# ssheybani/baby-vision-curriculum

Hardware: AMD Instinct MI355X
Metric: video clips/sec (node) VideoMAE-base 16x224^2 bf16 pretraining (higher is better)
Workload: dtype bf16; 1 GPU; VideoMAE-base (ViT-B/16 encoder, 4-layer decoder), 16x224x224 clips, tubelet 2, 90% tube mask, full training step (fwd + MSE + bwd + GradScaler + SGD-Nesterov); clips_per_gpu=256, global_batch=256, parallelism=dp1, weights=random init N(0,0.02), seed 0

## Files before the change

__graft_entry__.py:

```python
import importlib.util
import os
import subprocess
import sys

ROOT = os.path.dirname(os.path.abspath(__file__))
PKG_DIR = os.path.join(ROOT, "baby-vision-curriculum_amd")
CSRC = os.path.join(PKG_DIR, "csrc")
LIB = os.path.join(PKG_DIR, "libbvc_hip.so")
PRODUCT_SOURCES = ["gemm.hip", "gemm_persist.hip", "gemm8.hip", "gemm_as.hip", "attention.hip", "attention_probs.hip", "rowops.hip", "stack.hip", "videomae.hip", "jepa.hip", "comm.hip"]
EXPERIMENT_SOURCES = [os.path.join("experiments", "gemm_big.hip"), os.path.join("experiments", "gemm_pp.hip")]
EXPERIMENT_INCLUDES = [os.path.join("experiments", "attention_dq_wave96.inc")]
HEADERS = ["common.h", "dropgate.h", "gemm.h", "gemm_tile.h", "gemm_kernel_body.inc", "attention.h", "attention_fwd_body.inc", "attention_dq_body.inc", "attention_dkdv_body.inc", "rowops.h", "stack.h", os.path.join("..", "..", "include", "bvc.h")]


def _experiments():
    return "BVC_EXPERIMENTS" in os.environ.get("BVC_EXTRA_HIPCC_FLAGS", "")


def _sources():
    return PRODUCT_SOURCES + (EXPERIMENT_SOURCES if _experiments() else [])


SOURCES = PRODUCT_SOURCES


EXPERIMENT_FLAGS = {"attention.hip": ["-mllvm", "-amdgpu-mfma-vgpr-form=1"]}


def _extra_flags(src):
    return EXPERIMENT_FLAGS.get(src, []) if _experiments() else []


HASH_FILE = LIB + ".srchash"


def _source_hash():
    import hashlib
    h = hashlib.sha256()
    for f in _sources() + HEADERS + (EXPERIMENT_INCLUDES if _experiments() else []):
        with open(os.path.join(CSRC, f), "rb") as fh:
            h.update(f.encode() + b"\0" + fh.read())
    h.update(os.environ.get("BVC_EXTRA_HIPCC_FLAGS", "").encode())
    return h.hexdigest()


def _stale():
    if not (os.path.exists(LIB) and os.path.exists(HASH_FILE)):
        return True
    with open(HASH_FILE) as fh:
        return fh.read().strip() != _source_hash()


def _hash_of(files):
    import hashlib
    h = hashlib.sha256()
    for f in files:
        with open(os.path.join(CSRC, f), "rb") as fh:
            h.update(f.encode() + b"\0" + fh.read())
    return h.hexdigest()


def build(force: bool = False) -> None:
    if force or _stale():
        from concurrent.futures import ThreadPoolExecutor
        hipcc = os.environ.get("HIPCC", "/opt/rocm/bin/hipcc")
        objdir = os.path.join(PKG_DIR, "build")
        os.makedirs(objdir, exist_ok=True)
        flags = ["--offload-arch=gfx950", "-O3", "-std=c++17", "-fPIC"] + os.environ.get("BVC_EXTRA_HIPCC_FLAGS", "").split()

        def compile_one(src):
            obj = os.path.join(objdir, os.path.basename(src).replace(".hip", ".o"))
            stamp = obj + ".hash"
            fl = flags + _extra_flags(src) + ["-I" + CSRC]
            want = _hash_of([src] + HEADERS + (EXPERIMENT_INCLUDES if _experiments() else [])) + " " + " ".join(fl)
            if not force and os.path.exists(obj) and os.path.exists(stamp) and open(stamp).read() == want:
                return obj
            cmd = [hipcc, *fl, "-c", os.path.join(CSRC, src), "-o", obj]
            if src == "gemm8.hip":
                r = subprocess.run(cmd + ["-Rpass-analysis=kernel-resource-usage"], stderr=subprocess.PIPE, text=True)
                if r.returncode != 0:
                    sys.stderr.write(r.stderr)
                    raise subprocess.CalledProcessError(r.returncode, cmd)
                name = None
                for line in r.stderr.splitlines():
                    if "Function Name:" in line:
                        name = line.split("Function Name:")[1].split()[0]
                    elif "VGPRs Spill:" in line and name and "gemm8_kernel" in name and name.endswith("ELi0EEEvNS_9GemmGroupEi"):
                        if int(line.split("VGPRs Spill:")[1].split()[0]) != 0:
                            raise RuntimeError(f"gemm8.hip: {name} spills VGPRs; its counted-wait epilogue assumes none")
            else:
                subprocess.run(cmd, check=True)
            with open(stamp, "w") as fh:
                fh.write(want)
            return obj

        srcs = _sources()
        with ThreadPoolExecutor(max_workers=min(8, len(srcs))) as ex:
            objs = list(ex.map(compile_one, srcs))
        subprocess.run([hipcc, "--offload-arch=gfx950", "-shared", "-fPIC", *objs, "-o", LIB], check=True)
        with open(HASH_FILE, "w") as fh:
            fh.write(_source_hash())
    pkg = load_package()
    pkg._lib.lib()


def load_package():
    if "bvc_amd" in sys.modules:
        return sys.modules["bvc_amd"]
    spec = importlib.util.spec_from_file_location("bvc_amd", os.path.join(PKG_DIR, "__init__.py"),
                                                  submodule_search_locations=[PKG_DIR])
    mod = importlib.util.module_from_spec(spec)
    sys.modules["bvc_amd"] = mod
    spec.loader.exec_module(mod)
    return mod


def smoke() -> None:
    import torch
    if ROOT not in sys.path:
        sys.path.insert(0, ROOT)
    from oracle import videomae_oracle as vo
    build()
    bvc = load_package()
    cfg = vo.TINY
    params = vo.make_params(cfg, seed=0)
    pixels, mask = vo.synthetic_batch(cfg, 2, seed=0, mask_ratio=0.75)
    ref_loss, ref_grads = vo.step(cfg, params, pixels, mask)

    dev = torch.device("cuda:0")
    model = bvc.VideoMAEForPreTraining(bvc.VideoMAEConfig(**{k: v for k, v in cfg.__dict__.items() if k != "decoder_norm_eps"}))
    model.load_state_dict(params)
    model.to(dev).train()
    out = model(pixels.to(dev), bool_masked_pos=mask.to(dev))
    out.loss.backward()
    torch.cuda.synchronize()
    loss = float(out.loss)
    rel = abs(loss - float(ref_loss)) / abs(float(ref_loss))
    assert rel < 2e-3, f"smoke: loss {loss} vs oracle {float(ref_loss)} (rel {rel:.2e})"
    for name in vo.GRAD_PROBES:
        g = dict(model.named_parameters())[name].grad.float().cpu()
        r = ref_grads[name]
        e = float((g - r).norm() / r.norm())
        assert e < 3e-2, f"smoke: grad {name} rel err {e:.2e}"
    print(f"smoke ok: loss {loss:.6f} (oracle {float(ref_loss):.6f}, rel {rel:.1e})")


if __name__ == "__main__":
    build(force="--force" in sys.argv)
    if "--smoke" in sys.argv:
        smoke()
```

baby-vision-curriculum_amd/csrc/attention.hip:

```cpp
#include <stdlib.h>

#include "attention.h"

namespace bvc {

#define AS3 __attribute__((address_space(3)))
#define MFMA32(a, b, c) __builtin_amdgcn_mfma_f32_32x32x16_bf16((a), (b), (c), 0, 0, 0)

template <int HD>
__device__ __forceinline__ int swz_dual(int r) {
    if constexpr (HD == 64) return (((r >> 1) & 1) << 2) | ((r >> 2) & 3);
    else return (r >> 2) & 3;
}

template <int HD>
constexpr int pan_w(int p) { return HD - 64 * p >= 64 ? 64 : HD - 64 * p; }
constexpr int img_hd(int hd) { return hd == 80 || hd == 88 ? 96 : hd; }
constexpr uint32_t kDmaZero = 0xfffffff0u;
__device__ __forceinline__ int swz_pw(int pw, int r) { return pw == 64 ? swz_dual<64>(r) : swz_dual<32>(r); }

template <int PW, int NW, int VC = PW / 8>
__device__ __forceinline__ void stage_panel(__amdgpu_buffer_rsrc_t rs, int row0, int ld, int col0, char* lds, int GB, int wave, int lane) {
    constexpr int CPR = PW / 8;
    constexpr int RPP = 64 / CPR;
#pragma unroll
    for (int jj = 0; jj < (PW / 8 + NW - 1) / NW; ++jj) {
        const int j = wave + NW * jj;
        if (NW > PW / 8 && j >= PW / 8) break;
        const int r = RPP * j + lane / CPR;
        const int c = (lane % CPR) ^ swz_dual<PW>(r);
        uint32_t off = (uint32_t)(((size_t)(row0 + r) * ld + col0 + c * 8) * 2);
        if constexpr (VC < CPR) off = c < VC ? off : kDmaZero;
        const uint32_t dst = (uint32_t)((RPP * j >> 4) * GB + ((RPP * j) & 15) * PW * 2);
        glds16(rs, off, __builtin_amdgcn_readfirstlane((uint32_t)(size_t)((AS3 char*)lds) + dst));
    }
}

template <int HD, int NW = 4, int HV = HD>
__device__ __forceinline__ void stage64(__amdgpu_buffer_rsrc_t rs, int row0, int ld, int col0, char* lds,
                                        int wave, int lane) {
    static_assert(HV == HD || (HD == 96 && HV > 64 && HV % 8 == 0), "stage64: a narrower head only on the 96 image");
    if constexpr (HD > 64) {
        stage_panel<64, NW>(rs, row0, ld, col0, lds, 16 * HD * 2, wave, lane);
        stage_panel<pan_w<HD>(1), NW, (HV - 64) / 8>(rs, row0, ld, col0 + 64, lds + 2048, 16 * HD * 2, wave, lane);
        return;
    }
    constexpr int CPR = HD / 8;
    constexpr int RPP = 64 / CPR;
#pragma unroll
    for (int jj = 0; jj < (HD / 8 + NW - 1) / NW; ++jj) {
        const int j = wave + NW * jj;
        if (NW > HD / 8 && j >= HD / 8) break;
        const int r = RPP * j + lane / CPR;
        const int c = (lane % CPR) ^ swz_dual<HD>(r);
        const uint32_t off = (uint32_t)(((size_t)(row0 + r) * ld + col0 + c * 8) * 2);
        glds16(rs, off, __builtin_amdgcn_readfirstlane((uint32_t)(size_t)((AS3 char*)lds) + (uint32_t)j * 1024u));
    }
}

template <int HD>
struct FragAddr {
    uint32_t rows[HD / 16];
    uint32_t tr[HD / 32][2];
};

template <int HD>
__device__ __forceinline__ FragAddr<HD> make_frag_addr(int lane) {
    FragAddr<HD> a;
    if constexpr (HD > 64) {
        constexpr int GB = 16 * HD * 2;
        const int r = lane & 31, h = lane >> 5, rg = r & 15;
#pragma unroll
        for (int st = 0; st < HD / 16; ++st) {
            const int pw = pan_w<HD>(st >> 2);
            a.rows[st] = (r >> 4) * GB + (st >> 2) * 2048 + rg * pw * 2 + (((2 * (st & 3) + h) ^ swz_pw(pw, rg)) << 4);
        }
        const int q = (lane >> 2) & 3, p = lane & 3;
#pragma unroll
        for (int t = 0; t < HD / 32; ++t) {
            const int pw = pan_w<HD>(t >> 1);
            const int col = 32 * (t & 1) + 16 * ((lane >> 4) & 1) + 4 * p;
            const int chunk = col >> 3, within = (col & 7) * 2;
#pragma unroll
            for (int half = 0; half < 2; ++half) {
                const int r0 = 4 * h + q + 8 * half;
                a.tr[t][half] = (t >> 1) * 2048 + r0 * pw * 2 + ((chunk ^ swz_pw(pw, r0)) << 4) + within;
            }
        }
        return a;
    }
    constexpr int RB = HD * 2;
    const int r = lane & 31, h = lane >> 5;
#pragma unroll
    for (int st = 0; st < HD / 16; ++st) a.rows[st] = r * RB + (((2 * st + h) ^ swz_dual<HD>(r)) << 4);
    const int q = (lane >> 2) & 3, p = lane & 3;
#pragma unroll
    for (int t = 0; t < HD / 32; ++t) {
        const int col = 32 * t + 16 * ((lane >> 4) & 1) + 4 * p;
        const int chunk = col >> 3, within = (col & 7) * 2;
#pragma unroll
        for (int half = 0; half < 2; ++half) {
            const int r0 = 4 * h + q + 8 * half;
            a.tr[t][half] = r0 * RB + ((chunk ^ swz_dual<HD>(r0)) << 4) + within;
        }
    }
    return a;
}

template <int IMM>
__device__ __forceinline__ bf16x8 lds_rows(const AS3 char* base, uint32_t off) {
    return *reinterpret_cast<const AS3 bf16x8*>(base + off + IMM);
}

template <int IMM>
__device__ __forceinline__ bf16x8 lds_tr(const AS3 char* base, uint32_t off_lo, uint32_t off_hi) {
    const bf16x4 lo = __builtin_amdgcn_ds_read_tr16_b64_v4i16((AS3 bf16x4*)(base + off_lo + IMM));
    const bf16x4 hi = __builtin_amdgcn_ds_read_tr16_b64_v4i16((AS3 bf16x4*)(base + off_hi + IMM));
    return __builtin_shufflevector(lo, hi, 0, 1, 2, 3, 4, 5, 6, 7);
}

__device__ __forceinline__ bf16x8 acc_to_frag(const f32x16& a, int s) {
    union { bf16x8 v; uint32_t u[4]; } r;
#pragma unroll
    for (int j = 0; j < 4; ++j) r.u[j] = pack2bf(a[8 * s + 2 * j], a[8 * s + 2 * j + 1]);
    return r.v;
}

__device__ __forceinline__ int acc_row(int reg, int h) { return (reg & 3) + 8 * (reg >> 2) + 4 * h; }

__device__ __forceinline__ bf16x8 load8(const bf16_t* p) { return *reinterpret_cast<const bf16x8*>(p); }
template <int HV, int HI>
__device__ __forceinline__ bf16x8 load8_head(const bf16_t* p, int col) {
    if constexpr (HV == HI) return load8(p);
    else {
        const bf16x8 z = {0, 0, 0, 0, 0, 0, 0, 0};
        return col < HV ? load8(p) : z;
    }
}

template <typename T>
__device__ __forceinline__ void settle(T& v) { asm volatile("" : "+v"(v)); }

__device__ __forceinline__ f32x16 zero16() {
    f32x16 z;
#pragma unroll
    for (int i = 0; i < 16; ++i) z[i] = 0.f;
    return z;
}

__device__ __forceinline__ float xhalf_max(float v) {
    const auto r = __builtin_amdgcn_permlane32_swap(__float_as_uint(v), __float_as_uint(v), false, false);
    return fmaxf(__uint_as_float(r[0]), __uint_as_float(r[1]));
}
__device__ __forceinline__ float xhalf_sum(float v) {
    const auto r = __builtin_amdgcn_permlane32_swap(__float_as_uint(v), __float_as_uint(v), false, false);
    return __uint_as_float(r[0]) + __uint_as_float(r[1]);
}

__device__ __forceinline__ float fast_exp2(float x) { return __builtin_amdgcn_exp2f(x); }

constexpr float kDeferLog2 = 6.0f;

template <int HD>
struct FwdState {
    f32x16 o[HD / 32];
    float m_run, l_run;
};

template <int HD, int KOFF, int VOFF>
__device__ __forceinline__ void fwd_subtile(const AS3 char* lds, const FragAddr<HD>& fa, const bf16x8 (&qf)[HD / 16], FwdState<HD>& st,
                                            int key0, int N, int h, float scale_log2) {
    constexpr int KS = 16 * HD * 2;
    f32x16 s = zero16();
#pragma unroll
    for (int stp = 0; stp < HD / 16; ++stp) s = MFMA32(lds_rows<KOFF>(lds, fa.rows[stp]), qf[stp], s);
    if (key0 + 32 > N) {
        asm volatile("" ::: "memory");
#pragma unroll
        for (int r = 0; r < 16; ++r)
            if (key0 + acc_row(r, h) >= N) s[r] = -INFINITY;
    }
    float mx = s[0];
#pragma unroll
    for (int r = 1; r < 16; ++r) mx = fmaxf(mx, s[r]);
    mx = xhalf_max(mx) * scale_log2;
    if (!__all(mx - st.m_run <= kDeferLog2)) {
        const float m_new = fmaxf(st.m_run, mx);
        const float alpha = fast_exp2(st.m_run - m_new);
        st.m_run = m_new;
        st.l_run *= alpha;
#pragma unroll
        for (int t = 0; t < HD / 32; ++t)
#pragma unroll
            for (int r = 0; r < 16; ++r) st.o[t][r] *= alpha;
    }
    const float nm = -st.m_run;
    float rs = 0.f;
#pragma unroll
    for (int r = 0; r < 16; ++r) {
        s[r] = fast_exp2(fmaf(s[r], scale_log2, nm));
        rs += s[r];
    }
    st.l_run += rs;
    const bf16x8 p0 = acc_to_frag(s, 0), p1 = acc_to_frag(s, 1);
#pragma unroll
    for (int t = 0; t < HD / 32; ++t) st.o[t] = MFMA32(lds_tr<VOFF>(lds, fa.tr[t][0], fa.tr[t][1]), p0, st.o[t]);
#pragma unroll
    for (int t = 0; t < HD / 32; ++t) st.o[t] = MFMA32(lds_tr<VOFF + KS>(lds, fa.tr[t][0], fa.tr[t][1]), p1, st.o[t]);
}

__device__ __forceinline__ void attn_block(int tiles, int remap, int& tile, int& bh) {
    const int nb = gridDim.x, bid = blockIdx.x;
    int lid = bid;
    if (remap) {
        const int xq = nb >> 3, xr = nb & 7, xcd = bid & 7;
        lid = (xcd < xr ? xcd * (xq + 1) : xr * (xq + 1) + (xcd - xr) * xq) + (bid >> 3);
    }
    bh = lid / tiles;
    tile = lid - bh * tiles;
}

struct TailSplit { int gs, own, part, valid; };
template <int NW = 4>
__device__ __forceinline__ TailSplit tail_split(int N, int tile, int wave) {
    if constexpr (NW != 4) { TailSplit t; t.valid = NW; t.gs = 1; t.own = wave; t.part = 0; return t; }
    const int rows = N - tile * 128;
    TailSplit t;
    t.valid = rows >= 128 ? 4 : (rows + 31) >> 5;
    t.gs = t.valid == 1 ? 4 : t.valid == 2 ? 2 : 1;
    t.own = t.gs == 1 ? wave : wave & (t.valid - 1);
    t.part = t.gs == 1 ? 0 : wave >> (t.valid - 1);
    return t;
}
template <int NT>
__device__ __forceinline__ void tail_reduce(char* buf, const TailSplit& ts, int lane, f32x16 (&acc)[NT]) {
    AS3 float* cl = (AS3 float*)buf;
    constexpr int SLOT = NT * 16 * 64;
    __syncthreads();
    if (ts.part > 0) {
        AS3 float* w = cl + ((ts.part - 1) * ts.valid + ts.own) * SLOT + lane;
#pragma unroll
        for (int t = 0; t < NT; ++t)
#pragma unroll
            for (int r = 0; r < 16; ++r) w[(t * 16 + r) * 64] = acc[t][r];
    }
    __syncthreads();
    if (ts.part == 0) {
        for (int p = 1; p < ts.gs; ++p) {
            const AS3 float* w = cl + ((p - 1) * ts.valid + ts.own) * SLOT + lane;
#pragma unroll
            for (int t = 0; t < NT; ++t)
#pragma unroll
                for (int r = 0; r < 16; ++r) acc[t][r] += w[(t * 16 + r) * 64];
        }
    }
}


template <int HD, int NW = 4>
__global__ __launch_bounds__(64 * NW, 2) void attn_fwd_kernel(const bf16_t* __restrict__ qkv, bf16_t* __restrict__ ctx,
                                                          float* __restrict__ lse, int N, int H, int D,
                                                          uint32_t qkv_bytes, float scale_log2, int remap) {
    constexpr bool WIN = false;
    const int q_off_ = 0, Nq_ = N;
#include "attention_fwd_body.inc"
}
template <int HD>
__global__ __launch_bounds__(256, 2) void attn_fwd_win_kernel(const bf16_t* __restrict__ qkv, bf16_t* __restrict__ ctx,
                                                              float* __restrict__ lse, int N, int H, int D,
                                                              uint32_t qkv_bytes, float scale_log2, int remap, int q_off_, int Nq_) {
    constexpr bool WIN = true;
    constexpr int NW = 4;
#include "attention_fwd_body.inc"
}

template <int HD, int KOFF, int VOFF>
__device__ __forceinline__ void dq_subtile(const AS3 char* lds, const FragAddr<HD>& fa, const bf16x8 (&qf)[HD / 16],
                                           const bf16x8 (&dof)[HD / 16], f32x16 (&dq)[HD / 32], int key0, int N, int h,
                                           float scale_log2, float nlse, const f32x16& ndel) {
    constexpr int KS = 16 * HD * 2;
    f32x16 s = zero16(), dp;
#pragma unroll
    for (int stp = 0; stp < HD / 16; ++stp) {
        s = MFMA32(lds_rows<KOFF>(lds, fa.rows[stp]), qf[stp], s);
        dp = MFMA32(lds_rows<VOFF>(lds, fa.rows[stp]), dof[stp], stp == 0 ? ndel : dp);
    }
#pragma unroll
    for (int r = 0; r < 16; ++r)
        s[r] = fast_exp2(fmaf(s[r], scale_log2, nlse)) * dp[r];
    if (key0 + 32 > N) {
        asm volatile("" ::: "memory");
#pragma unroll
        for (int r = 0; r < 16; ++r)
            if (key0 + acc_row(r, h) >= N) s[r] = 0.f;
    }
    const bf16x8 d0 = acc_to_frag(s, 0), d1 = acc_to_frag(s, 1);
#pragma unroll
    for (int t = 0; t < HD / 32; ++t) dq[t] = MFMA32(lds_tr<KOFF>(lds, fa.tr[t][0], fa.tr[t][1]), d0, dq[t]);
#pragma unroll
    for (int t = 0; t < HD / 32; ++t) dq[t] = MFMA32(lds_tr<KOFF + KS>(lds, fa.tr[t][0], fa.tr[t][1]), d1, dq[t]);
}


template <int HD>
__global__ __launch_bounds__(256, 2) void attn_bwd_dq_kernel(const bf16_t* __restrict__ qkv, const bf16_t* __restrict__ dctx,
                                                             const bf16_t* __restrict__ ctx, const float* __restrict__ lse,
                                                             float* __restrict__ delta, bf16_t* __restrict__ dqkv, int N, int H, int D,
                                                             uint32_t qkv_bytes, float scale, float scale_log2, int remap) {
    constexpr bool WIN = false;
    const int q_off_ = 0, Nq_ = N;
#include "attention_dq_body.inc"
}
template <int HD>
__global__ __launch_bounds__(256, 2) void attn_bwd_dq_win_kernel(const bf16_t* __restrict__ qkv, const bf16_t* __restrict__ dctx,
                                                                 const bf16_t* __restrict__ ctx, const float* __restrict__ lse,
                                                                 float* __restrict__ delta, bf16_t* __restrict__ dqkv, int N, int H, int D,
                                                                 uint32_t qkv_bytes, float scale, float scale_log2, int remap, int q_off_, int Nq_) {
    constexpr bool WIN = true;
#include "attention_dq_body.inc"
}

#ifdef BVC_EXPERIMENTS
#include "experiments/attention_dq_wave96.inc"
#endif

template <int HD, int QOFF, int STAT>
__device__ __forceinline__ void dkdv_subtile(const AS3 char* lds, const FragAddr<HD>& fa, const bf16x8 (&kf)[HD / 16],
                                             const bf16x8 (&vf)[HD / 16], f32x16 (&dk)[HD / 32], f32x16 (&dv)[HD / 32], int q0,
                                             int N, int h, float scale_log2) {
    constexpr int IMG = 64 * HD * 2, KS = 16 * HD * 2;
    constexpr int DOFF = QOFF + IMG;
#ifndef BVC_ATTN_STATS_LDS
    bf16x8 sfrag, one_s, one_d;
    {
        const AS3 float* st = reinterpret_cast<const AS3 float*>(lds + STAT);
        const int r = threadIdx.x & 31;
        const float xl = -st[r] * (1.0f / scale_log2), xd = st[64 + r];
        const uint32_t hh = pack2bf(xl, xd);
        const float lhi = __uint_as_float(hh << 16), dhi = __uint_as_float(hh & 0xffff0000u);
        const uint32_t ll = pack2bf(xl - lhi, xd - dhi);
        union { bf16x8 v; uint32_t u[4]; } f, a, b;
        f.u[0] = h ? 0u : ((hh & 0xffffu) | (ll << 16));
        f.u[1] = h ? 0u : ((hh >> 16) | (ll & 0xffff0000u));
        f.u[2] = 0u; f.u[3] = 0u;
        a.u[0] = h ? 0u : 0x3f803f80u; a.u[1] = 0u; a.u[2] = 0u; a.u[3] = 0u;
        b.u[0] = 0u; b.u[1] = h ? 0u : 0x3f803f80u; b.u[2] = 0u; b.u[3] = 0u;
        sfrag = f.v; one_s = a.v; one_d = b.v;
    }
    f32x16 s = zero16(), dp = zero16();
#pragma unroll
    for (int stp = 0; stp < HD / 16; ++stp) {
        s = MFMA32(lds_rows<QOFF>(lds, fa.rows[stp]), kf[stp], s);
        dp = MFMA32(lds_rows<DOFF>(lds, fa.rows[stp]), vf[stp], dp);
    }
    s = MFMA32(sfrag, one_s, s);
    dp = MFMA32(sfrag, one_d, dp);
#pragma unroll
    for (int r = 0; r < 16; ++r) {
        const float p = fast_exp2(s[r] * scale_log2);
        s[r] = p;
        dp[r] = p * dp[r];
    }
#else
    const AS3 float* stl = reinterpret_cast<const AS3 float*>(lds + STAT) + 4 * h;
    f32x16 s = zero16(), dp;
#pragma unroll
    for (int g = 0; g < 4; ++g) {
        const f32x4 nd = *reinterpret_cast<const AS3 f32x4*>(stl + 64 + 8 * g);
#pragma unroll
        for (int e = 0; e < 4; ++e) dp[4 * g + e] = nd[e];
    }
#pragma unroll
    for (int stp = 0; stp < HD / 16; ++stp) {
        s = MFMA32(lds_rows<QOFF>(lds, fa.rows[stp]), kf[stp], s);
        dp = MFMA32(lds_rows<DOFF>(lds, fa.rows[stp]), vf[stp], dp);
    }
#pragma unroll
    for (int g = 0; g < 4; ++g) {
        const f32x4 ls = *reinterpret_cast<const AS3 f32x4*>(stl + 8 * g);
#pragma unroll
        for (int e = 0; e < 4; ++e) {
            const int r = 4 * g + e;
            const float p = fast_exp2(fmaf(s[r], scale_log2, -ls[e]));
            s[r] = p;
            dp[r] = p * dp[r];
        }
    }
#endif
    if (q0 + 32 > N) {
        asm volatile("" ::: "memory");
#pragma unroll
        for (int r = 0; r < 16; ++r)
            if (q0 + acc_row(r, h) >= N) { s[r] = 0.f; dp[r] = 0.f; }
    }
    const bf16x8 p0 = acc_to_frag(s, 0), p1 = acc_to_frag(s, 1);
    const bf16x8 d0 = acc_to_frag(dp, 0), d1 = acc_to_frag(dp, 1);
#pragma unroll
    for (int t = 0; t < HD / 32; ++t) {
        dv[t] = MFMA32(lds_tr<DOFF>(lds, fa.tr[t][0], fa.tr[t][1]), p0, dv[t]);
        dk[t] = MFMA32(lds_tr<QOFF>(lds, fa.tr[t][0], fa.tr[t][1]), d0, dk[t]);
    }
#pragma unroll
    for (int t = 0; t < HD / 32; ++t) {
        dv[t] = MFMA32(lds_tr<DOFF + KS>(lds, fa.tr[t][0], fa.tr[t][1]), p1, dv[t]);
        dk[t] = MFMA32(lds_tr<QOFF + KS>(lds, fa.tr[t][0], fa.tr[t][1]), d1, dk[t]);
    }
}


template <int HD>
__global__ __launch_bounds__(256, img_hd(HD) > 96 ? 1 : 2) void attn_bwd_dkdv_kernel(const bf16_t* __restrict__ qkv, const bf16_t* __restrict__ dctx,
                                                               const float* __restrict__ lse, const float* __restrict__ delta,
                                                               bf16_t* __restrict__ dqkv, int N, int H, int D,
                                                               uint32_t qkv_bytes, uint32_t dctx_bytes, uint32_t stat_bytes,
                                                               float scale, float scale_log2, int remap) {
    constexpr bool WIN = false;
    const int q_off_ = 0, Nq_ = N;
#include "attention_dkdv_body.inc"
}
template <int HD>
__global__ __launch_bounds__(256, img_hd(HD) > 96 ? 1 : 2) void attn_bwd_dkdv_win_kernel(const bf16_t* __restrict__ qkv, const bf16_t* __restrict__ dctx,
                                                               const float* __restrict__ lse, const float* __restrict__ delta,
                                                               bf16_t* __restrict__ dqkv, int N, int H, int D,
                                                               uint32_t qkv_bytes, uint32_t dctx_bytes, uint32_t stat_bytes,
                                                               float scale, float scale_log2, int remap, int q_off_, int Nq_) {
    constexpr bool WIN = true;
#include "attention_dkdv_body.inc"
}

template <int HD, int NBT>
__global__ __launch_bounds__(320, 1) void attn_bwd_head_kernel(const bf16_t* __restrict__ qkv, const bf16_t* __restrict__ dctx,
                                                               const bf16_t* __restrict__ ctx, const float* __restrict__ lse,
                                                               bf16_t* __restrict__ dqkv, int N, int H, int D, int nheads,
                                                               uint32_t qkv_bytes, uint32_t dctx_bytes, float scale, float scale_log2) {
    static_assert(HD == 64, "whole-head backward: head_dim 64");
    extern __shared__ __attribute__((aligned(16))) char smem[];
    constexpr int IMG = 192 * HD * 2, SUB = 32 * HD * 2, KS = 16 * HD * 2;
    constexpr int QI = 0, KI = IMG, VI = 2 * IMG, OI = 3 * IMG;
    constexpr int STAT = 4 * IMG;
    constexpr int DST = STAT + 2 * 192 * 4;
    const AS3 char* lds = (const AS3 char*)smem;
    const int tid = threadIdx.x, lane = tid & 63;
    const int wave = __builtin_amdgcn_readfirstlane(tid >> 6);
    const int ld = 3 * D, h = lane >> 5;
    const int NB = NBT > 0 ? NBT : (N + 31) >> 5;
    const __amdgpu_buffer_rsrc_t rq = make_rsrc(qkv, qkv_bytes), rd = make_rsrc(dctx, dctx_bytes);
    const FragAddr<HD> fa = make_frag_addr<HD>(lane);
    const FragAddr<32> fs = make_frag_addr<32>(lane);

    auto stage_qvo = [&](int bh) __attribute__((always_inline)) {
        if (wave < 4) {
            const int b = bh / H, head = bh % H, row0 = b * N;
            for (int rb = 0; rb * 64 < N; ++rb) {
                stage64<HD>(rq, row0 + rb * 64, ld, head * HD, smem + QI + rb * 2 * SUB, wave, lane);
                stage64<HD>(rq, row0 + rb * 64, ld, 2 * D + head * HD, smem + VI + rb * 2 * SUB, wave, lane);
                stage64<HD>(rd, row0 + rb * 64, D, head * HD, smem + OI + rb * 2 * SUB, wave, lane);
            }
        }
    };
    auto stage_k = [&](int bh) __attribute__((always_inline)) {
        if (wave < 4) {
            const int b = bh / H, head = bh % H, row0 = b * N;
            for (int rb = 0; rb * 64 < N; ++rb) stage64<HD>(rq, row0 + rb * 64, ld, D + head * HD, smem + KI + rb * 2 * SUB, wave, lane);
        }
    };
    float st_lse = 0.f, st_del[5];
    auto load_stats = [&](int bh) __attribute__((always_inline)) {
        const int b = bh / H, head = bh % H;
        st_lse = (tid < N) ? lse[(size_t)bh * N + tid] : 0.f;
#pragma unroll
        for (int k = 0; k < 5; ++k) {
            const int q = (tid >> 3) + 40 * k, c = tid & 7;
            float acc = 0.f;
            if (q < N) {
                const bf16x8 dv = load8(dctx + (size_t)(b * N + q) * D + head * HD + 8 * c);
                const bf16x8 ov = load8(ctx + (size_t)(b * N + q) * D + head * HD + 8 * c);
#pragma unroll
                for (int j = 0; j < 8; ++j) acc += bf2f((bf16_t)dv[j]) * bf2f((bf16_t)ov[j]);
            }
            st_del[k] = acc;
        }
    };
    auto store_stats = [&]() __attribute__((always_inline)) {
        AS3 float* st = (AS3 float*)((AS3 char*)smem + STAT);
        if (tid < 192) st[tid] = st_lse;
#pragma unroll
        for (int k = 0; k < 5; ++k) {
            float acc = st_del[k];
            acc += __shfl_xor(acc, 1, 64);
            acc += __shfl_xor(acc, 2, 64);
            acc += __shfl_xor(acc, 4, 64);
            const int q = (tid >> 3) + 40 * k;
            if ((tid & 7) == 0 && q < 192) st[192 + q] = -acc;
        }
    };

    int bh = blockIdx.x;
    if (bh >= nheads) return;
    load_stats(bh);
    stage_qvo(bh);
    stage_k(bh);
    for (; bh < nheads; bh += gridDim.x) {
    const int b = bh / H, head = bh % H;
    const int nxt = bh + gridDim.x;
    asm volatile("s_waitcnt vmcnt(0)" ::: "memory");
    store_stats();
    __syncthreads();

    for (int kb = wave; kb < NB; kb += 5) {
        const int ki = kb * 32 + (lane & 31);
        bf16x8 kf[HD / 16], vf[HD / 16];
#pragma unroll
        for (int st = 0; st < HD / 16; ++st) {
            kf[st] = *reinterpret_cast<const AS3 bf16x8*>(lds + KI + kb * SUB + fa.rows[st]);
            vf[st] = *reinterpret_cast<const AS3 bf16x8*>(lds + VI + kb * SUB + fa.rows[st]);
        }
        f32x16 dk[HD / 32], dv[HD / 32];
#pragma unroll
        for (int t = 0; t < HD / 32; ++t) { dk[t] = zero16(); dv[t] = zero16(); }
        const bool key_ok = ki < N;
#pragma unroll
        for (int qb = 0; qb < (NBT > 0 ? NBT : NB); ++qb) {
            const AS3 char* qim = lds + QI + qb * SUB;
            const AS3 char* oim = lds + OI + qb * SUB;
            const AS3 float* stl = reinterpret_cast<const AS3 float*>(lds + STAT) + qb * 32 + 4 * h;
            f32x16 s = zero16(), dp;
#pragma unroll
            for (int g = 0; g < 4; ++g) {
                const f32x4 nd = *reinterpret_cast<const AS3 f32x4*>(stl + 192 + 8 * g);
#pragma unroll
                for (int e = 0; e < 4; ++e) dp[4 * g + e] = nd[e];
            }
#pragma unroll
            for (int stp = 0; stp < HD / 16; ++stp) {
                s = MFMA32(*reinterpret_cast<const AS3 bf16x8*>(qim + fa.rows[stp]), kf[stp], s);
                dp = MFMA32(*reinterpret_cast<const AS3 bf16x8*>(oim + fa.rows[stp]), vf[stp], dp);
            }
#pragma unroll
            for (int g = 0; g < 4; ++g) {
                const f32x4 ls = *reinterpret_cast<const AS3 f32x4*>(stl + 8 * g);
#pragma unroll
                for (int e = 0; e < 4; ++e) {
                    const int r = 4 * g + e;
                    const float pr = fast_exp2(fmaf(s[r], scale_log2, -ls[e]));
                    s[r] = pr;
                    dp[r] = pr * dp[r];
                }
            }
            if (qb * 32 + 32 > N || !__all(key_ok)) {
                asm volatile("" ::: "memory");
#pragma unroll
                for (int r = 0; r < 16; ++r)
                    if (!key_ok || qb * 32 + acc_row(r, h) >= N) { s[r] = 0.f; dp[r] = 0.f; }
            }
            const bf16x8 p0 = acc_to_frag(s, 0), p1 = acc_to_frag(s, 1);
            const bf16x8 d0 = acc_to_frag(dp, 0), d1 = acc_to_frag(dp, 1);
            {
                AS3 char* blk = (AS3 char*)smem + DST + (kb * 5 + qb) * 2048 + (lane & 31) * 64 + 8 * h;
                const int sw = swz_dual<32>(lane & 31);
                typedef __attribute__((ext_vector_type(2))) unsigned int u32x2;
                union { bf16x8 v; u32x2 u[2]; } w0, w1;
                w0.v = d0; w1.v = d1;
                *reinterpret_cast<AS3 u32x2*>(blk + ((0 ^ sw) << 4)) = w0.u[0];
                *reinterpret_cast<AS3 u32x2*>(blk + ((1 ^ sw) << 4)) = w0.u[1];
                *reinterpret_cast<AS3 u32x2*>(blk + ((2 ^ sw) << 4)) = w1.u[0];
                *reinterpret_cast<AS3 u32x2*>(blk + ((3 ^ sw) << 4)) = w1.u[1];
            }
#pragma unroll
            for (int t = 0; t < HD / 32; ++t) {
                dv[t] = MFMA32(lds_tr<0>(oim, fa.tr[t][0], fa.tr[t][1]), p0, dv[t]);
                dk[t] = MFMA32(lds_tr<0>(qim, fa.tr[t][0], fa.tr[t][1]), d0, dk[t]);
            }
#pragma unroll
            for (int t = 0; t < HD / 32; ++t) {
                dv[t] = MFMA32(lds_tr<KS>(oim, fa.tr[t][0], fa.tr[t][1]), p1, dv[t]);
                dk[t] = MFMA32(lds_tr<KS>(qim, fa.tr[t][0], fa.tr[t][1]), d1, dk[t]);
            }
        }
        if (key_ok) {
            bf16_t* krow = dqkv + (size_t)(b * N + ki) * ld + D + head * HD;
            bf16_t* vrow = krow + D;
#pragma unroll
            for (int t = 0; t < HD / 32; ++t)
#pragma unroll
                for (int g = 0; g < 4; ++g) {
                    const int d = 32 * t + 8 * g + 4 * h;
                    uint2 a = {pack2bf(dk[t][4 * g] * scale, dk[t][4 * g + 1] * scale), pack2bf(dk[t][4 * g + 2] * scale, dk[t][4 * g + 3] * scale)};
                    *reinterpret_cast<uint2*>(krow + d) = a;
                    uint2 e = {pack2bf(dv[t][4 * g], dv[t][4 * g + 1]), pack2bf(dv[t][4 * g + 2], dv[t][4 * g + 3])};
                    *reinterpret_cast<uint2*>(vrow + d) = e;
                }
        }
    }
    __syncthreads();
    if (nxt < nheads) {
        stage_qvo(nxt);
        load_stats(nxt);
    }

    for (int qb = wave; qb < NB; qb += 5) {
        const int qi = qb * 32 + (lane & 31);
        f32x16 dq[HD / 32];
#pragma unroll
        for (int t = 0; t < HD / 32; ++t) dq[t] = zero16();
#pragma unroll
        for (int kb = 0; kb < (NBT > 0 ? NBT : NB); ++kb) {
            const AS3 char* kim = lds + KI + kb * SUB;
            const AS3 char* blk = lds + DST + (kb * 5 + qb) * 2048;
            const bf16x8 b0 = lds_tr<0>(blk, fs.tr[0][0], fs.tr[0][1]);
            const bf16x8 b1 = lds_tr<1024>(blk, fs.tr[0][0], fs.tr[0][1]);
#pragma unroll
            for (int t = 0; t < HD / 32; ++t) dq[t] = MFMA32(lds_tr<0>(kim, fa.tr[t][0], fa.tr[t][1]), b0, dq[t]);
#pragma unroll
            for (int t = 0; t < HD / 32; ++t) dq[t] = MFMA32(lds_tr<KS>(kim, fa.tr[t][0], fa.tr[t][1]), b1, dq[t]);
        }
        if (qi < N) {
            bf16_t* orow = dqkv + (size_t)(b * N + qi) * ld + head * HD;
#pragma unroll
            for (int t = 0; t < HD / 32; ++t)
#pragma unroll
                for (int g = 0; g < 4; ++g) {
                    const int d = 32 * t + 8 * g + 4 * h;
                    uint2 a = {pack2bf(dq[t][4 * g] * scale, dq[t][4 * g + 1] * scale), pack2bf(dq[t][4 * g + 2] * scale, dq[t][4 * g + 3] * scale)};
                    *reinterpret_cast<uint2*>(orow + d) = a;
                }
        }
    }
    __syncthreads();
    if (nxt < nheads) stage_k(nxt);
    }
}

static int xcd_remap() {
#ifdef BVC_EXPERIMENTS
    return getenv("BVC_ATTN_PLAIN_GRID") == nullptr;
#else
    return 1;
#endif
}

static bool head_kernel_enabled() {
#ifdef BVC_EXPERIMENTS
    return getenv("BVC_ATTN_NO_HEAD_KERNEL") == nullptr;
#else
    return true;
#endif
}

template <int HD>
static int fwd_hd(const bf16_t* qkv, bf16_t* ctx, float* lse, int B, int N, int H, hipStream_t stream, float sm_scale) {
    constexpr int HI = img_hd(HD);
    const int D = H * HD;
    const size_t bytes = (size_t)B * N * 3 * D * 2;
    const float scale_log2 = (sm_scale > 0.f ? sm_scale : 1.0f / sqrtf((float)HD)) * 1.4426950408889634f;
#ifdef BVC_EXPERIMENTS
    if (getenv("BVC_ATTN_NW8") != nullptr) {
        const dim3 grid8((unsigned)(((N + 255) / 256) * B * H));
        hipLaunchKernelGGL((attn_fwd_kernel<HD, 8>), grid8, dim3(512), 4 * 64 * HI * 2, stream, qkv, ctx, lse, N, H, D, (uint32_t)bytes, scale_log2,
                           xcd_remap());
        BVC_CHECK_HIP(hipGetLastError());
        return BVC_OK;
    }
#endif
    const dim3 grid((unsigned)(((N + 127) / 128) * B * H));
    hipLaunchKernelGGL((attn_fwd_kernel<HD, 4>), grid, dim3(256), 4 * 64 * HI * 2, stream, qkv, ctx, lse, N, H, D, (uint32_t)bytes, scale_log2,
                       xcd_remap());
    BVC_CHECK_HIP(hipGetLastError());
    return BVC_OK;
}

template <int HD>
static int bwd_hd(const bf16_t* qkv, const bf16_t* ctx, const bf16_t* dctx, const float* lse, float* delta, bf16_t* dqkv, int B,
                  int N, int H, hipStream_t stream, float sm_scale, int parts) {
    constexpr int HI = img_hd(HD);
    const int D = H * HD;
    const size_t bytes = (size_t)B * N * 3 * D * 2;
    const float scale = sm_scale > 0.f ? sm_scale : 1.0f / sqrtf((float)HD), scale_log2 = scale * 1.4426950408889634f;
    const dim3 grid((unsigned)(((N + 127) / 128) * B * H));
    const int remap = xcd_remap();
    if constexpr (HD == 64) {
        if (parts == 3 && N <= 160 && head_kernel_enabled()) {
            constexpr size_t lds = 4 * 192 * HD * 2 + 2 * 192 * 4 + 25 * 2048;
            static bool attr_set = false;
            if (!attr_set) {
                BVC_CHECK_HIP(hipFuncSetAttribute(reinterpret_cast<const void*>(&attn_bwd_head_kernel<HD, 5>),
                                                  hipFuncAttributeMaxDynamicSharedMemorySize, (int)lds));
                BVC_CHECK_HIP(hipFuncSetAttribute(reinterpret_cast<const void*>(&attn_bwd_head_kernel<HD, 0>),
                                                  hipFuncAttributeMaxDynamicSharedMemorySize, (int)lds));
                attr_set = true;
            }
            static int ncu = 0;
            if (ncu == 0) {
                int dev = 0;
                hipDeviceProp_t prop;
                BVC_CHECK_HIP(hipGetDevice(&dev));
                BVC_CHECK_HIP(hipGetDeviceProperties(&prop, dev));
                ncu = prop.multiProcessorCount > 0 ? prop.multiProcessorCount : 256;
            }
            const int nheads = B * H;
            const dim3 g((unsigned)(nheads < ncu ? nheads : ncu));
            if (N > 128)
                hipLaunchKernelGGL((attn_bwd_head_kernel<HD, 5>), g, dim3(320), lds, stream, qkv, dctx, ctx, lse, dqkv, N, H, D, nheads,
                                   (uint32_t)bytes, (uint32_t)((size_t)B * N * D * 2), scale, scale_log2);
            else
                hipLaunchKernelGGL((attn_bwd_head_kernel<HD, 0>), g, dim3(320), lds, stream, qkv, dctx, ctx, lse, dqkv, N, H, D, nheads,
                                   (uint32_t)bytes, (uint32_t)((size_t)B * N * D * 2), scale, scale_log2);
            BVC_CHECK_HIP(hipGetLastError());
            return BVC_OK;
        }
    }
    if (parts & 1) {
#ifdef BVC_EXPERIMENTS
    if (HI == HD && getenv("BVC_ATTN_DQ_W") != nullptr) {
        constexpr int NB = 3;
        const dim3 gridw((unsigned)(((N + 32 * NB - 1) / (32 * NB)) * B * H));
        hipLaunchKernelGGL((attn_bwd_dq_w_kernel<HI, NB>), gridw, dim3(64), kRing * 2 * 32 * HI * 2, stream, qkv, dctx, ctx, lse, delta, dqkv, N, H, D,
                           (uint32_t)bytes, scale, scale_log2, remap);
    } else
#endif
    hipLaunchKernelGGL(attn_bwd_dq_kernel<HD>, grid, dim3(256), 4 * 64 * HI * 2, stream, qkv, dctx, ctx, lse, delta, dqkv, N, H, D,
                       (uint32_t)bytes, scale, scale_log2, remap);
    }
    if (parts & 2) {
    constexpr int lds_dkdv = 2 * (2 * 64 * HI * 2 + 512);
    if constexpr (lds_dkdv > 65536) {
        static bool attr_set = false;
        if (!attr_set) {
            BVC_CHECK_HIP(hipFuncSetAttribute(reinterpret_cast<const void*>(&attn_bwd_dkdv_kernel<HD>),
                                              hipFuncAttributeMaxDynamicSharedMemorySize, lds_dkdv));
            attr_set = true;
        }
    }
    hipLaunchKernelGGL(attn_bwd_dkdv_kernel<HD>, grid, dim3(256), lds_dkdv, stream, qkv, dctx, lse, delta, dqkv, N, H, D,
                       (uint32_t)bytes, (uint32_t)((size_t)B * N * D * 2), (uint32_t)((size_t)B * H * N * 4), scale, scale_log2, remap);
    }
    BVC_CHECK_HIP(hipGetLastError());
    return BVC_OK;
}

static bool attn_hd_ok(int hd) { return hd == 32 || hd == 64 || hd == 80 || hd == 88 || hd == 96 || hd == 128; }

int launch_attn_fwd(const bf16_t* qkv, bf16_t* ctx, float* lse, int B, int N, int H, int head_dim, hipStream_t stream, float sm_scale) {
    BVC_REQUIRE(B > 0 && N > 0 && H > 0, "attn_fwd: empty shape");
    BVC_REQUIRE(attn_hd_ok(head_dim), "attn_fwd: head_dim %d unsupported (32, 64, 80, 88, 96 or 128)", head_dim);
    BVC_REQUIRE((size_t)B * N * 3 * H * head_dim * 2 < 0xffffffffull, "attn_fwd: qkv larger than 4 GiB");
    BVC_REQUIRE(img_hd(head_dim) == head_dim || (size_t)B * N * 3 * H * head_dim * 2 < kDmaZero,
                "attn_fwd: qkv of head_dim %d must stay below 4 GiB - 16 bytes", head_dim);
    switch (head_dim) {
        case 32: return fwd_hd<32>(qkv, ctx, lse, B, N, H, stream, sm_scale);
        case 80: return fwd_hd<80>(qkv, ctx, lse, B, N, H, stream, sm_scale);
        case 88: return fwd_hd<88>(qkv, ctx, lse, B, N, H, stream, sm_scale);
        case 96: return fwd_hd<96>(qkv, ctx, lse, B, N, H, stream, sm_scale);
        case 128: return fwd_hd<128>(qkv, ctx, lse, B, N, H, stream, sm_scale);
        default: return fwd_hd<64>(qkv, ctx, lse, B, N, H, stream, sm_scale);
    }
}

int launch_attn_bwd(const bf16_t* qkv, const bf16_t* ctx, const bf16_t* dctx, const float* lse, float* delta,
                    bf16_t* dqkv, int B, int N, int H, int head_dim, hipStream_t stream, float sm_scale, int parts) {
    BVC_REQUIRE(B > 0 && N > 0 && H > 0, "attn_bwd: empty shape");
    BVC_REQUIRE(attn_hd_ok(head_dim), "attn_bwd: head_dim %d unsupported (32, 64, 80, 88, 96 or 128)", head_dim);
    BVC_REQUIRE((size_t)B * N * 3 * H * head_dim * 2 < 0xffffffffull, "attn_bwd: qkv larger than 4 GiB");
    BVC_REQUIRE(img_hd(head_dim) == head_dim || (size_t)B * N * 3 * H * head_dim * 2 < kDmaZero,
                "attn_bwd: qkv of head_dim %d must stay below 4 GiB - 16 bytes", head_dim);
    switch (head_dim) {
        case 32: return bwd_hd<32>(qkv, ctx, dctx, lse, delta, dqkv, B, N, H, stream, sm_scale, parts);
        case 80: return bwd_hd<80>(qkv, ctx, dctx, lse, delta, dqkv, B, N, H, stream, sm_scale, parts);
        case 88: return bwd_hd<88>(qkv, ctx, dctx, lse, delta, dqkv, B, N, H, stream, sm_scale, parts);
        case 96: return bwd_hd<96>(qkv, ctx, dctx, lse, delta, dqkv, B, N, H, stream, sm_scale, parts);
        case 128: return bwd_hd<128>(qkv, ctx, dctx, lse, delta, dqkv, B, N, H, stream, sm_scale, parts);
        default: return bwd_hd<64>(qkv, ctx, dctx, lse, delta, dqkv, B, N, H, stream, sm_scale, parts);
    }
}

bool attn_window_ok(int head_dim) { return head_dim == 64; }

int launch_attn_fwd_win(const bf16_t* qkv, bf16_t* ctx, float* lse, int B, int N, int H, int head_dim, int q_off, int Nq, hipStream_t stream,
                        float sm_scale) {
    BVC_REQUIRE(B > 0 && N > 0 && H > 0, "attn_fwd_win: empty shape");
    BVC_REQUIRE(attn_window_ok(head_dim), "attn_fwd_win: head_dim %d has no query-window kernel (64)", head_dim);
    BVC_REQUIRE(q_off >= 0 && Nq > 0 && q_off + Nq <= N, "attn_fwd_win: window (%d, %d) outside the %d rows", q_off, Nq, N);
    BVC_REQUIRE((size_t)B * N * 3 * H * head_dim * 2 < 0xffffffffull, "attn_fwd_win: qkv larger than 4 GiB");
    constexpr int HD = 64;
    const int D = H * HD;
    const float scale_log2 = (sm_scale > 0.f ? sm_scale : 1.0f / sqrtf((float)HD)) * 1.4426950408889634f;
    const dim3 grid((unsigned)(((Nq + 127) / 128) * B * H));
    hipLaunchKernelGGL(attn_fwd_win_kernel<HD>, grid, dim3(256), 4 * 64 * HD * 2, stream, qkv, ctx, lse, N, H, D,
                       (uint32_t)((size_t)B * N * 3 * D * 2), scale_log2, xcd_remap(), q_off, Nq);
    BVC_CHECK_HIP(hipGetLastError());
    return BVC_OK;
}

int launch_attn_bwd_win(const bf16_t* qkv, const bf16_t* ctx, const bf16_t* dctx, const float* lse, float* delta, bf16_t* dqkv, int B, int N,
                        int H, int head_dim, int q_off, int Nq, hipStream_t stream, float sm_scale) {
    BVC_REQUIRE(B > 0 && N > 0 && H > 0, "attn_bwd_win: empty shape");
    BVC_REQUIRE(attn_window_ok(head_dim), "attn_bwd_win: head_dim %d has no query-window kernel (64)", head_dim);
    BVC_REQUIRE(q_off >= 0 && Nq > 0 && q_off + Nq == N, "attn_bwd_win: the window (%d, %d) must end with the %d rows", q_off, Nq, N);
    BVC_REQUIRE((size_t)B * N * 3 * H * head_dim * 2 < 0xffffffffull, "attn_bwd_win: qkv larger than 4 GiB");
    constexpr int HD = 64;
    const int D = H * HD;
    const uint32_t bytes = (uint32_t)((size_t)B * N * 3 * D * 2);
    const float scale = sm_scale > 0.f ? sm_scale : 1.0f / sqrtf((float)HD), scale_log2 = scale * 1.4426950408889634f;
    const int remap = xcd_remap();
    const dim3 gq((unsigned)((((q_off + 127) / 128) + ((Nq + 127) / 128)) * B * H));
    hipLaunchKernelGGL(attn_bwd_dq_win_kernel<HD>, gq, dim3(256), 4 * 64 * HD * 2, stream, qkv, dctx, ctx, lse, delta, dqkv, N, H, D, bytes,
                       scale, scale_log2, remap, q_off, Nq);
    const dim3 gk((unsigned)(((N + 127) / 128) * B * H));
    hipLaunchKernelGGL(attn_bwd_dkdv_win_kernel<HD>, gk, dim3(256), 2 * (2 * 64 * HD * 2 + 512), stream, qkv, dctx, lse, delta, dqkv, N, H, D, bytes,
                       (uint32_t)((size_t)B * Nq * D * 2), (uint32_t)((size_t)B * H * Nq * 4), scale, scale_log2, remap, q_off, Nq);
    BVC_CHECK_HIP(hipGetLastError());
    return BVC_OK;
}

}
```

Baseline: 3368 clips/s.

## Double-buffer Q/dO staging in whole-head attention backward with counted vmcnt waits

Restructures the persistent whole-head attention backward kernel so the next head's Q and dO images are staged into a second LDS slot while the current head computes. K/V fragments and stats now go straight into registers via global loads rather than through LDS. Full vmcnt(0) drains are replaced with counted waits, and dQ stores move to buffer stores. The aim is to hide global-load latency across heads and cut barrier stalls. In exchange it adds LDS double-buffering, fragile counted waits (guarded at build time by a scratch-usage check), and an experiment-only ablation knob.

```diff
diff --git a/__graft_entry__.py b/__graft_entry__.py
--- a/__graft_entry__.py
+++ b/__graft_entry__.py
@@ -88,6 +88,18 @@
                     elif "VGPRs Spill:" in line and name and "gemm8_kernel" in name and name.endswith("ELi0EEEvNS_9GemmGroupEi"):
                         if int(line.split("VGPRs Spill:")[1].split()[0]) != 0:
                             raise RuntimeError(f"gemm8.hip: {name} spills VGPRs; its counted-wait epilogue assumes none")
+            elif src == "attention.hip":
+                r = subprocess.run(cmd + ["-Rpass-analysis=kernel-resource-usage"], stderr=subprocess.PIPE, text=True)
+                if r.returncode != 0:
+                    sys.stderr.write(r.stderr)
+                    raise subprocess.CalledProcessError(r.returncode, cmd)
+                name = None
+                for line in r.stderr.splitlines():
+                    if "Function Name:" in line:
+                        name = line.split("Function Name:")[1].split()[0]
+                    elif "ScratchSize [bytes/lane]:" in line and name and "attn_bwd_head_kernel" in name:
+                        if int(line.split("ScratchSize [bytes/lane]:")[1].split()[0]) != 0:
+                            raise RuntimeError(f"attention.hip: {name} uses scratch; its counted waits assume none")
             else:
                 subprocess.run(cmd, check=True)
             with open(stamp, "w") as fh:
diff --git a/baby-vision-curriculum_amd/csrc/attention.hip b/baby-vision-curriculum_amd/csrc/attention.hip
--- a/baby-vision-curriculum_amd/csrc/attention.hip
+++ b/baby-vision-curriculum_amd/csrc/attention.hip
@@ -428,106 +428,160 @@
 #include "attention_dkdv_body.inc"
 }
 
+#ifndef BVC_EXP_ENV
+#ifdef BVC_EXPERIMENTS
+#define BVC_EXP_ENV(name) getenv(name)
+#else
+#define BVC_EXP_ENV(name) ((const char*)nullptr)
+#endif
+#endif
+
+__device__ __forceinline__ void wait_vmcnt(int n) {
+#define BVC_VMW(k) case k: asm volatile("s_waitcnt vmcnt(" #k ")" ::: "memory"); break;
+    switch (n) {
+        BVC_VMW(8) BVC_VMW(16)
+        BVC_VMW(17) BVC_VMW(19) BVC_VMW(21) BVC_VMW(23) BVC_VMW(25) BVC_VMW(27)
+        BVC_VMW(33) BVC_VMW(35) BVC_VMW(37) BVC_VMW(39) BVC_VMW(41) BVC_VMW(43)
+        default: asm volatile("s_waitcnt vmcnt(0)" ::: "memory");
+    }
+#undef BVC_VMW
+}
+
 template <int HD, int NBT>
 __global__ __launch_bounds__(320, 1) void attn_bwd_head_kernel(const bf16_t* __restrict__ qkv, const bf16_t* __restrict__ dctx,
                                                                const bf16_t* __restrict__ ctx, const float* __restrict__ lse,
                                                                bf16_t* __restrict__ dqkv, int N, int H, int D, int nheads,
-                                                               uint32_t qkv_bytes, uint32_t dctx_bytes, float scale, float scale_log2) {
+                                                               uint32_t qkv_bytes, uint32_t dctx_bytes, float scale, float scale_log2,
+                                                               int abl_) {
     static_assert(HD == 64, "whole-head backward: head_dim 64");
     extern __shared__ __attribute__((aligned(16))) char smem[];
-    constexpr int IMG = 192 * HD * 2, SUB = 32 * HD * 2, KS = 16 * HD * 2;
-    constexpr int QI = 0, KI = IMG, VI = 2 * IMG, OI = 3 * IMG;
-    constexpr int STAT = 4 * IMG;
-    constexpr int DST = STAT + 2 * 192 * 4;
+    constexpr int ROWS = 160;
+    constexpr int IMG = ROWS * HD * 2, SUB = 32 * HD * 2, KS = 16 * HD * 2;
+    constexpr int KI = 0, QI = IMG, OI = 3 * IMG;
+    constexpr int DST = 5 * IMG;
+    constexpr int STAT = DST + 25 * 2048, STATB = 2 * ROWS * 4;
+    constexpr int NST1 = 2 * (HD / 32) * 4, NST2 = (HD / 32) * 4;
+    constexpr int NLD = 2 * (HD / 16) + 1 + 2 * 4;
+#ifdef BVC_EXPERIMENTS
+    const int abl = abl_;
+#else
+    constexpr int abl = 0;
+#endif
     const AS3 char* lds = (const AS3 char*)smem;
     const int tid = threadIdx.x, lane = tid & 63;
     const int wave = __builtin_amdgcn_readfirstlane(tid >> 6);
     const int ld = 3 * D, h = lane >> 5;
     const int NB = NBT > 0 ? NBT : (N + 31) >> 5;
+    const int P = (N + 7) >> 3;
+    const int npc = wave < 4 ? (P - wave + 3) >> 2 : 0;
     const __amdgpu_buffer_rsrc_t rq = make_rsrc(qkv, qkv_bytes), rd = make_rsrc(dctx, dctx_bytes);
     const FragAddr<HD> fa = make_frag_addr<HD>(lane);
     const FragAddr<32> fs = make_frag_addr<32>(lane);
 
-    auto stage_qvo = [&](int bh) __attribute__((always_inline)) {
-        if (wave < 4) {
-            const int b = bh / H, head = bh % H, row0 = b * N;
-            for (int rb = 0; rb * 64 < N; ++rb) {
-                stage64<HD>(rq, row0 + rb * 64, ld, head * HD, smem + QI + rb * 2 * SUB, wave, lane);
-                stage64<HD>(rq, row0 + rb * 64, ld, 2 * D + head * HD, smem + VI + rb * 2 * SUB, wave, lane);
-                stage64<HD>(rd, row0 + rb * 64, D, head * HD, smem + OI + rb * 2 * SUB, wave, lane);
-            }
-        }
+    auto stage_img = [&](__amdgpu_buffer_rsrc_t rs, int row0, int ldr, int col0, int dst) __attribute__((always_inline)) {
+        if (wave < 4)
+            for (int j = wave; j < P; j += 4) {
+                const int r = 8 * j + (lane >> 3);
+                const int c = (lane & 7) ^ swz_dual<HD>(r);
+                const uint32_t off = (uint32_t)(((size_t)(row0 + r) * ldr + col0 + c * 8) * 2);
+                glds16(rs, off, __builtin_amdgcn_readfirstlane((uint32_t)(size_t)((AS3 char*)smem) + (uint32_t)dst + (uint32_t)j * 1024u));
+            }
     };
-    auto stage_k = [&](int bh) __attribute__((always_inline)) {
-        if (wave < 4) {
-            const int b = bh / H, head = bh % H, row0 = b * N;
-            for (int rb = 0; rb * 64 < N; ++rb) stage64<HD>(rq, row0 + rb * 64, ld, D + head * HD, smem + KI + rb * 2 * SUB, wave, lane);
-        }
+    auto stage_qo = [&](int bhx, int slot) __attribute__((always_inline)) {
+        const int b = bhx / H, head = bhx % H;
+        stage_img(rq, b * N, ld, head * HD, QI + slot * IMG);
+        stage_img(rd, b * N, D, head * HD, OI + slot * IMG);
     };
-    float st_lse = 0.f, st_del[5];
-    auto load_stats = [&](int bh) __attribute__((always_inline)) {
-        const int b = bh / H, head = bh % H;
-        st_lse = (tid < N) ? lse[(size_t)bh * N + tid] : 0.f;
-#pragma unroll
-        for (int k = 0; k < 5; ++k) {
-            const int q = (tid >> 3) + 40 * k, c = tid & 7;
+    auto stage_k = [&](int bhx) __attribute__((always_inline)) { stage_img(rq, (bhx / H) * N, ld, D + (bhx % H) * HD, KI); };
+    bf16x8 kf[HD / 16], vf[HD / 16];
+    const int kc = min(wave * 32 + (lane & 31), N - 1);
+    auto load_kv = [&](int bhx) __attribute__((always_inline)) {
+        const bf16_t* krow = qkv + (size_t)((bhx / H) * N + kc) * ld + D + (bhx % H) * HD + 8 * h;
+#pragma unroll
+        for (int st = 0; st < HD / 16; ++st) {
+            kf[st] = load8(krow + 16 * st);
+            vf[st] = load8(krow + D + 16 * st);
+        }
+    };
+    float st_lse = 0.f;
+    bf16x8 st_do[4], st_o[4];
+    auto load_stats = [&](int bhx) __attribute__((always_inline)) {
+        const int b = bhx / H, head = bhx % H;
+        st_lse = lse[(size_t)bhx * N + min(tid, N - 1)];
+#pragma unroll
+        for (int k = 0; k < 4; ++k) {
+            const size_t at = (size_t)(b * N + min((tid >> 3) + 40 * k, N - 1)) * D + head * HD + 8 * (tid & 7);
+            st_do[k] = load8(dctx + at);
+            st_o[k] = load8(ctx + at);
+        }
+    };
+    auto store_stats = [&](int slot) __attribute__((always_inline)) {
+        AS3 float* st = (AS3 float*)((AS3 char*)smem + STAT + slot * STATB);
+        if (tid < ROWS) st[tid] = tid < N ? st_lse : 0.f;
+#pragma unroll
+        for (int k = 0; k < 4; ++k) {
+            const int q = (tid >> 3) + 40 * k;
             float acc = 0.f;
-            if (q < N) {
-                const bf16x8 dv = load8(dctx + (size_t)(b * N + q) * D + head * HD + 8 * c);
-                const bf16x8 ov = load8(ctx + (size_t)(b * N + q) * D + head * HD + 8 * c);
-#pragma unroll
-                for (int j = 0; j < 8; ++j) acc += bf2f((bf16_t)dv[j]) * bf2f((bf16_t)ov[j]);
-            }
-            st_del[k] = acc;
-        }
-    };
-    auto store_stats = [&]() __attribute__((always_inline)) {
-        AS3 float* st = (AS3 float*)((AS3 char*)smem + STAT);
-        if (tid < 192) st[tid] = st_lse;
-#pragma unroll
-        for (int k = 0; k < 5; ++k) {
-            float acc = st_del[k];
+#pragma unroll
+            for (int j = 0; j < 8; ++j) acc += bf2f((bf16_t)st_do[k][j]) * bf2f((bf16_t)st_o[k][j]);
+            acc = q < N ? acc : 0.f;
             acc += __shfl_xor(acc, 1, 64);
             acc += __shfl_xor(acc, 2, 64);
             acc += __shfl_xor(acc, 4, 64);
-            const int q = (tid >> 3) + 40 * k;
-            if ((tid & 7) == 0 && q < 192) st[192 + q] = -acc;
+            if ((tid & 7) == 0) st[ROWS + q] = -acc;
         }
     };
 
     int bh = blockIdx.x;
     if (bh >= nheads) return;
+    load_kv(bh);
     load_stats(bh);
-    stage_qvo(bh);
-    stage_k(bh);
+    stage_qo(bh, 0);
+    {
+        typedef __attribute__((ext_vector_type(4))) unsigned int u32x4;
+        const u32x4 z = {0u, 0u, 0u, 0u};
+        for (int img = 0; img < 5; ++img)
+            for (int o = P * 1024 + tid * 16; o < NB * SUB; o += 320 * 16) *reinterpret_cast<AS3 u32x4*>((AS3 char*)smem + img * IMG + o) = z;
+    }
+    asm volatile("s_waitcnt vmcnt(0)" ::: "memory");
+#pragma unroll
+    for (int st = 0; st < HD / 16; ++st) { settle(kf[st]); settle(vf[st]); }
+    settle(st_lse);
+#pragma unroll
+    for (int k = 0; k < 4; ++k) { settle(st_do[k]); settle(st_o[k]); }
+    const __amdgpu_buffer_rsrc_t rg = make_rsrc(dqkv, qkv_bytes);
+    int slot = 0;
     for (; bh < nheads; bh += gridDim.x) {
     const int b = bh / H, head = bh % H;
     const int nxt = bh + gridDim.x;
-    asm volatile("s_waitcnt vmcnt(0)" ::: "memory");
-    store_stats();
+    const bool first = bh == (int)blockIdx.x;
+    const bool more = nxt < nheads && abl != 1;
+    const bool st_ok = abl != 1 || first;
+    const bool mine = NBT == 5 || wave < NB;
+    store_stats(slot);
     __syncthreads();
 
-    for (int kb = wave; kb < NB; kb += 5) {
+    if (st_ok) stage_k(bh);
+    if (more) stage_qo(nxt, slot ^ 1);
+    const AS3 char* qs = lds + QI + slot * IMG;
+    const AS3 float* sts = reinterpret_cast<const AS3 float*>(lds + STAT + slot * STATB);
+    if (mine) {
+        const int kb = wave;
         const int ki = kb * 32 + (lane & 31);
-        bf16x8 kf[HD / 16], vf[HD / 16];
-#pragma unroll
-        for (int st = 0; st < HD / 16; ++st) {
-            kf[st] = *reinterpret_cast<const AS3 bf16x8*>(lds + KI + kb * SUB + fa.rows[st]);
-            vf[st] = *reinterpret_cast<const AS3 bf16x8*>(lds + VI + kb * SUB + fa.rows[st]);
-        }
         f32x16 dk[HD / 32], dv[HD / 32];
 #pragma unroll
         for (int t = 0; t < HD / 32; ++t) { dk[t] = zero16(); dv[t] = zero16(); }
         const bool key_ok = ki < N;
+        if (abl != 2)
 #pragma unroll
         for (int qb = 0; qb < (NBT > 0 ? NBT : NB); ++qb) {
-            const AS3 char* qim = lds + QI + qb * SUB;
-            const AS3 char* oim = lds + OI + qb * SUB;
-            const AS3 float* stl = reinterpret_cast<const AS3 float*>(lds + STAT) + qb * 32 + 4 * h;
+            const AS3 char* qim = qs + qb * SUB;
+            const AS3 char* oim = qim + (OI - QI);
+            const AS3 float* stl = sts + qb * 32 + 4 * h;
             f32x16 s = zero16(), dp;
 #pragma unroll
             for (int g = 0; g < 4; ++g) {
-                const f32x4 nd = *reinterpret_cast<const AS3 f32x4*>(stl + 192 + 8 * g);
+                const f32x4 nd = *reinterpret_cast<const AS3 f32x4*>(stl + ROWS + 8 * g);
 #pragma unroll
                 for (int e = 0; e < 4; ++e) dp[4 * g + e] = nd[e];
             }
@@ -577,7 +631,7 @@
                 dk[t] = MFMA32(lds_tr<KS>(qim, fa.tr[t][0], fa.tr[t][1]), d1, dk[t]);
             }
         }
-        if (key_ok) {
+        if (st_ok && key_ok) {
             bf16_t* krow = dqkv + (size_t)(b * N + ki) * ld + D + head * HD;
             bf16_t* vrow = krow + D;
 #pragma unroll
@@ -592,17 +646,20 @@
                 }
         }
     }
+    if (more) {
+        load_kv(nxt);
+        load_stats(nxt);
+    }
+    wait_vmcnt((mine && st_ok ? NST1 : 0) + (more ? 2 * npc + NLD : 0));
     __syncthreads();
-    if (nxt < nheads) {
-        stage_qvo(nxt);
-        load_stats(nxt);
-    }
-
-    for (int qb = wave; qb < NB; qb += 5) {
+
+    if (mine) {
+        const int qb = wave;
         const int qi = qb * 32 + (lane & 31);
         f32x16 dq[HD / 32];
 #pragma unroll
         for (int t = 0; t < HD / 32; ++t) dq[t] = zero16();
+        if (abl != 2)
 #pragma unroll
         for (int kb = 0; kb < (NBT > 0 ? NBT : NB); ++kb) {
             const AS3 char* kim = lds + KI + kb * SUB;
@@ -614,20 +671,25 @@
 #pragma unroll
             for (int t = 0; t < HD / 32; ++t) dq[t] = MFMA32(lds_tr<KS>(kim, fa.tr[t][0], fa.tr[t][1]), b1, dq[t]);
         }
-        if (qi < N) {
-            bf16_t* orow = dqkv + (size_t)(b * N + qi) * ld + head * HD;
-#pragma unroll
-            for (int t = 0; t < HD / 32; ++t)
-#pragma unroll
-                for (int g = 0; g < 4; ++g) {
-                    const int d = 32 * t + 8 * g + 4 * h;
-                    uint2 a = {pack2bf(dq[t][4 * g] * scale, dq[t][4 * g + 1] * scale), pack2bf(dq[t][4 * g + 2] * scale, dq[t][4 * g + 3] * scale)};
-                    *reinterpret_cast<uint2*>(orow + d) = a;
-                }
-        }
-    }
-    __syncthreads();
-    if (nxt < nheads) stage_k(nxt);
+        const bool q_ok = st_ok && qi < N;
+        const uint32_t orow = (uint32_t)(((size_t)(b * N + qi) * ld + head * HD) * 2);
+#pragma unroll
+        for (int t = 0; t < HD / 32; ++t)
+#pragma unroll
+            for (int g = 0; g < 4; ++g) {
+                const int d = 32 * t + 8 * g + 4 * h;
+                typedef __attribute__((ext_vector_type(2))) unsigned int u32x2;
+                const u32x2 a = {pack2bf(dq[t][4 * g] * scale, dq[t][4 * g + 1] * scale), pack2bf(dq[t][4 * g + 2] * scale, dq[t][4 * g + 3] * scale)};
+                __builtin_amdgcn_raw_buffer_store_b64(a, rg, q_ok ? orow + 2u * d : kDmaZero, 0, 0);
+            }
+    }
+    if (abl != 1) slot ^= 1;
+    wait_vmcnt(mine ? NST2 : 0);
+#pragma unroll
+    for (int st = 0; st < HD / 16; ++st) { settle(kf[st]); settle(vf[st]); }
+    settle(st_lse);
+#pragma unroll
+    for (int k = 0; k < 4; ++k) { settle(st_do[k]); settle(st_o[k]); }
     }
 }
 
@@ -680,7 +742,7 @@
     const int remap = xcd_remap();
     if constexpr (HD == 64) {
         if (parts == 3 && N <= 160 && head_kernel_enabled()) {
-            constexpr size_t lds = 4 * 192 * HD * 2 + 2 * 192 * 4 + 25 * 2048;
+            constexpr size_t lds = 5 * 160 * HD * 2 + 25 * 2048 + 2 * 2 * 160 * 4;
             static bool attr_set = false;
             if (!attr_set) {
                 BVC_CHECK_HIP(hipFuncSetAttribute(reinterpret_cast<const void*>(&attn_bwd_head_kernel<HD, 5>),
@@ -698,13 +760,15 @@
                 ncu = prop.multiProcessorCount > 0 ? prop.multiProcessorCount : 256;
             }
             const int nheads = B * H;
+            const char* abl_e = BVC_EXP_ENV("BVC_ATTN_HEAD_ABL");
+            const int abl = abl_e ? atoi(abl_e) : 0;
             const dim3 g((unsigned)(nheads < ncu ? nheads : ncu));
             if (N > 128)
                 hipLaunchKernelGGL((attn_bwd_head_kernel<HD, 5>), g, dim3(320), lds, stream, qkv, dctx, ctx, lse, dqkv, N, H, D, nheads,
-                                   (uint32_t)bytes, (uint32_t)((size_t)B * N * D * 2), scale, scale_log2);
+                                   (uint32_t)bytes, (uint32_t)((size_t)B * N * D * 2), scale, scale_log2, abl);
             else
                 hipLaunchKernelGGL((attn_bwd_head_kernel<HD, 0>), g, dim3(320), lds, stream, qkv, dctx, ctx, lse, dqkv, N, H, D, nheads,
-                                   (uint32_t)bytes, (uint32_t)((size_t)B * N * D * 2), scale, scale_log2);
+                                   (uint32_t)bytes, (uint32_t)((size_t)B * N * D * 2), scale, scale_log2, abl);
             BVC_CHECK_HIP(hipGetLastError());
             return BVC_OK;
         }
```

Result: no change. 3396 clips/s (median of 3 runs) (+0.8%).
